# AutonomousVehicleLaboratory/vision_semantic_segmentation

Hardware: AMD Instinct MI355X
Metric: fused frames/sec/GPU (1920x1080 + 120k pts) + max|dlog-odds| vs ref (higher is better)
Workload: dtype f16 hi+lo split, MX-FP4 correction passes, fp32 accumulate

## Files before the change

### include/avl_hip.h

```cpp
#ifndef AVL_HIP_H
#define AVL_HIP_H

#include <stdint.h>

#ifdef __cplusplus
extern "C" {
#endif

#define AVL_OK 0
#define AVL_E_ARG (-1)
#define AVL_E_HIP (-2)
#define AVL_E_UNSUPPORTED (-3)

#define AVL_F32 0
#define AVL_F64 1
#define AVL_BF16 2
#define AVL_F16 3

#define AVL_MAX_MAP_CLASSES 16

const char* avl_version(void);
int avl_last_error(char* buf, int len);


// ... 252 lines not shown
    int32_t bias_per_image;
    int32_t in_format;
    int32_t raw_batch;
    void* out2;
    void* out2_lo;
    int32_t out2_ld, n_split;
} avl_seg_op;

#define AVL_IN_U8_HWC 0
#define AVL_IN_F32_CHW 1

#define AVL_MX_IN_LO 1
#define AVL_MX_RES_LO 2
#define AVL_MX_OUT_LO 4

typedef struct avl_seg_plan avl_seg_plan;

int avl_seg_plan_create(const avl_seg_op* ops_host, int n_ops, avl_seg_plan** out_plan);
void avl_seg_plan_destroy(avl_seg_plan* plan);
int avl_seg_plan_run(avl_seg_plan* plan, void* stream);
int avl_seg_plan_capture(avl_seg_plan* plan, void* stream);
int avl_seg_plan_profile(avl_seg_plan* plan, void* stream, float* ms_host, double* flops_host, double* bytes_host);
int avl_seg_plan_num_ops(const avl_seg_plan* plan);
int avl_seg_plan_nonfinite(avl_seg_plan* plan, void* stream, unsigned long long* counts_host);

#define AVL_GEMM_PLAIN 0
#define AVL_GEMM_RING 1
#define AVL_GEMM_RING_MX 2
#define AVL_GEMM_MX_PIPE 3

typedef struct avl_gemm_route {
    int32_t kernel;
    int32_t dtype;
    int32_t tile_m, tile_n;
    int32_t wm, wn;
    int32_t mi;
    int32_t stages;
    int32_t nsub;
    int32_t io;
    int32_t ast;
    int32_t ext;
    int32_t late;
    int32_t launches;
    int32_t m_tiles, n_tiles;
    int32_t workgroups;
} avl_gemm_route;
// ... 8 lines not shown
```

### vision_semantic_segmentation_amd/csrc/seg_conv.hip

```cpp
#include "seg_types.h"
#include "seg_preprocess.h"

namespace avl {
namespace {

constexpr int kThreads = 256;

template <typename T, bool F32IN = false>
__global__ void __launch_bounds__(kThreads) k_stem(const unsigned char* __restrict__ img, int H, int W,
                                                  const float* __restrict__ w, const float* __restrict__ bias,
                                                  T* __restrict__ out, int OH, int OW, int out_ld) {
    const int idx = blockIdx.x * kThreads + threadIdx.x;
    if (idx >= OH * OW) return;
    img = image_base(img, (long long)H * W, F32IN ? 3 * (int)sizeof(float) : 3);
    out = image_base(out, (long long)OH * OW, out_ld);
    const int oy = idx / OW, ox = idx % OW;
    float acc[64];
#pragma unroll
    for (int c = 0; c < 64; ++c) acc[c] = bias[c];
    const float mean[3] = {0.485f, 0.456f, 0.406f}, stdv[3] = {0.229f, 0.224f, 0.225f};
    for (int ky = 0; ky < 7; ++ky) {
        const int iy = oy * 2 - 3 + ky;
        for (int kx = 0; kx < 7; ++kx) {
            const int ix = ox * 2 - 3 + kx;
// ... 426 lines not shown
            Vec8<T>::load(in + (long long)(r + G) * in_ld + c8 * 8, v1);
            Vec8<T>::load(in + (long long)(r + 2 * G) * in_ld + c8 * 8, v2);
            Vec8<T>::load(in + (long long)(r + 3 * G) * in_ld + c8 * 8, v3);
#pragma unroll
            for (int i = 0; i < 8; ++i) s[i] += (v0[i] + v1[i]) + (v2[i] + v3[i]);
        }
        for (; r < M; r += G) {
            float v[8];
            Vec8<T>::load(in + (long long)r * in_ld + c8 * 8, v);
#pragma unroll
            for (int i = 0; i < 8; ++i) s[i] += v[i];
        }
        Vec8<float>::store(partial + (long long)blockIdx.x * C + c8 * 8, s);
    }
}
__global__ void __launch_bounds__(kThreads) k_gap_final(const float* __restrict__ partial, int G, int C, int M,
                                                       float* __restrict__ out, int out_ld) {
    __shared__ float red[8][32];
    const int cl = threadIdx.x & 31, sl = threadIdx.x >> 5;
    const int c = blockIdx.x * 32 + cl;
    partial = image_base(partial, G, C);
    out = image_base(out, 1, out_ld);
    float s = 0.f;
    if (c < C)
        for (int g = sl; g < G; g += 8) s += partial[(long long)g * C + c];
    red[sl][cl] = s;
    __syncthreads();
    if (sl == 0 && c < C) {
        float t = 0.f;
#pragma unroll
        for (int k = 0; k < 8; ++k) t += red[k][cl];
        out[c] = t / (float)M;
    }
}

__global__ void __launch_bounds__(kThreads) k_gemv(const float* __restrict__ in, const float* __restrict__ w,
                                                  const float* __restrict__ bias, float* __restrict__ out, int N, int K, int relu,
                                                  int in_ld, int out_ld) {
    const int n = blockIdx.x * (kThreads / 64) + (threadIdx.x >> 6);
    const int lane = threadIdx.x & 63;
    if (n >= N) return;
    in = image_base(in, 1, in_ld);
    out = image_base(out, 1, out_ld);
    const float* wr = w + (long long)n * K;
    float s0 = 0.f, s1 = 0.f, s2 = 0.f, s3 = 0.f;
    if ((K & 3) == 0 && (reinterpret_cast<uintptr_t>(wr) & 15) == 0 && (reinterpret_cast<uintptr_t>(in) & 15) == 0) {
#pragma unroll 8
        for (int k = lane * 4; k < K; k += 256) {
// ... 372 lines not shown
```

### vision_semantic_segmentation_amd/csrc/seg_dwpw.hip

```cpp
#include "seg_types.h"

namespace avl {
namespace {

constexpr int TM = 128;
constexpr int TN = 256;
constexpr int A_STAGE = TM * 128;
constexpr int W_STAGE = TN * 128;
constexpr int LDS_W = 0, LDS_A = 2 * W_STAGE, LDS_P = LDS_A + 2 * A_STAGE;
constexpr int P_STEP = 8 * 6 * 8 * 4;

struct DwPwArgs {
    const void* X;
    const void* X_lo;
    const void* Wc;
    const float* bc;
    float* LG;
    unsigned char* labels;
    int ncls;
    int tiles_x;
    const void* W;
    const float* bias;
    const uint32_t* dwp;
    const int* order;
// ... 184 lines not shown
                        hi[nj * 4 + r] = fmaxf(acc[mi][2 + nj][r], 0.f);
                    }
                HT* cp = static_cast<HT*>(p.C) + (long long)m * p.ldc + nbase;
                Vec8<HT>::store(cp, lo);
                Vec8<HT>::store(cp + 8, hi);
                if constexpr (WSUB != 1) {
                    if (p.C_lo) {
#pragma unroll
                        for (int i = 0; i < 8; ++i) { lo[i] -= (float)(HT)lo[i]; hi[i] -= (float)(HT)hi[i]; }
                        HT* cl = static_cast<HT*>(p.C_lo) + (long long)m * p.ldc + nbase;
                        Vec8<HT>::store(cl, lo);
                        Vec8<HT>::store(cl + 8, hi);
                    }
                }
            }
        }
    }
}

constexpr int X_LDS_W = 0, X_LDS_AH = 2 * W_STAGE, X_LDS_AL = X_LDS_AH + 2 * A_STAGE, X_LDS_P = X_LDS_AL + A_STAGE;
constexpr int XP_RING = 4;
constexpr int FP_STEP = 8 * 10 * 8 * 4;

__global__ void __launch_bounds__(512) k_dwpw_x(DwPwArgs p) {
    constexpr int PSTEP = FP_STEP;
    typedef f16 HT;
    typedef typename Half16<HT>::v8 v8;
    extern __shared__ __attribute__((aligned(16))) char lds[];
    const int tid = threadIdx.x, lane = tid & 63;
    const int wave = __builtin_amdgcn_readfirstlane(tid >> 6);
    const int wm = wave >> 2, wn = wave & 3;
    const int nt = blockIdx.x % p.ntiles;
    const int bm = blockIdx.x / p.ntiles, slot = (bm & 7) * p.per_xcd + (bm >> 3);
    if (slot >= p.mtiles) return;
    dwpw_image(p);
    const int mt = p.order[slot];
    const int nk = p.K / 64;

    const uint4* psrc = reinterpret_cast<const uint4*>(p.dwp);
    uint4 pnext = make_uint4(0u, 0u, 0u, 0u);
    auto load_p = [&](int s) { if (tid < PSTEP / 16 && s < nk) pnext = psrc[s * (PSTEP / 16) + tid]; };
    auto store_p = [&](int s) { if (tid < PSTEP / 16 && s < nk) *reinterpret_cast<uint4*>(lds + X_LDS_P + (s & (XP_RING - 1)) * PSTEP + tid * 16) = pnext; };
    for (int s = 0; s < 3; ++s) { load_p(s); store_p(s); }

    const int chunk = tid & 7, r0 = tid >> 3;
    unsigned voff[2][9];
#pragma unroll
    for (int q = 0; q < 2; ++q) {
        const int m = mt * TM + r0 + q * 64;
        const int y = m / p.OW, x = m - y * p.OW;
#pragma unroll
        for (int t = 0; t < 9; ++t) {
            const int iy = y - p.pad + (t / 3) * p.dil, ix = x - p.pad + (t % 3) * p.dil;
            const bool ok = m < p.M && iy >= 0 && iy < p.H && ix >= 0 && ix < p.Wd;
            voff[q][t] = ok ? (unsigned)(((long long)iy * p.Wd + ix) * p.ldx + chunk * 8) * 2u : 0x7fffff00u;
        }
    }
    const int wchunk = tid & 7, wrow0 = tid >> 3;
    const __amdgpu_buffer_rsrc_t wrsrc = __builtin_amdgcn_make_buffer_rsrc(
        const_cast<char*>(static_cast<const char*>(p.W) + (long long)nt * TN * p.K * 4), 0, TN * p.K * 4, 0x00020000);
    int w_voff[4];
#pragma unroll
    for (int i = 0; i < 4; ++i) w_voff[i] = (wrow0 + 64 * i) * p.K * 4 + wchunk * 16;
    v4i wl[4];
    auto load_w = [&](int h) {
#pragma unroll
        for (int i = 0; i < 4; ++i) wl[i] = __builtin_amdgcn_raw_buffer_load_b128(wrsrc, w_voff[i], h * 128, 0);
    };
    auto store_w = [&](int h) {
#pragma unroll
        for (int i = 0; i < 4; ++i) {
            const int r = wrow0 + 64 * i;
            const int key = ((r >> 1) & 1) | (((r >> 4) & 3) << 1);
            *reinterpret_cast<v4i*>(lds + X_LDS_W + (h & 1) * W_STAGE + r * 128 + ((wchunk ^ key) << 4)) = wl[i];
        }
// ... 8 lines not shown
        a_key[mi] = row & 7;
    }
#pragma unroll
    for (int nj = 0; nj < 4; ++nj) {
        const int row = wn * 64 + (fr >> 2) * 16 + nj * 4 + (fr & 3);
        w_off[nj] = X_LDS_W + row * 128;
        w_key[nj] = ((row >> 1) & 1) | (((row >> 4) & 3) << 1);
    }
    f32x4 acc[4][4];
    {
        const int nb = nt * TN + wn * 64 + kq * 16;
#pragma unroll
        for (int nj = 0; nj < 4; ++nj) {
            const float4 b = *reinterpret_cast<const float4*>(p.bias + nb + 4 * nj);
#pragma unroll
            for (int mi = 0; mi < 4; ++mi) acc[mi][nj] = f32x4{b.x, b.y, b.z, b.w};
        }
    }

    v4i raw[2][9];
    const __amdgpu_buffer_rsrc_t xrsrc = __builtin_amdgcn_make_buffer_rsrc(const_cast<void*>(p.X), 0, (int)p.x_bytes, 0x00020000);
    auto load_taps = [&](int s, int q) {
#pragma unroll
        for (int t = 0; t < 9; ++t) raw[q][t] = __builtin_amdgcn_raw_buffer_load_b128(xrsrc, (int)voff[q][t], s * 128, 0);
    };

    auto produce_a = [&](int s, int q) {
        float o[8];
        const float* pf = reinterpret_cast<const float*>(lds + X_LDS_P + (s & (XP_RING - 1)) * PSTEP + chunk * (10 * 8 * 4));
        {
            const float4 b0 = *reinterpret_cast<const float4*>(pf + 9 * 8), b1 = *reinterpret_cast<const float4*>(pf + 9 * 8 + 4);
            o[0] = b0.x; o[1] = b0.y; o[2] = b0.z; o[3] = b0.w;
            o[4] = b1.x; o[5] = b1.y; o[6] = b1.z; o[7] = b1.w;
        }
        typedef _Float16 h2 __attribute__((ext_vector_type(2)));
#pragma unroll
        for (int t = 0; t < 9; ++t) {
            const float4 w0 = *reinterpret_cast<const float4*>(pf + t * 8), w1 = *reinterpret_cast<const float4*>(pf + t * 8 + 4);
            const float wt[8] = {w0.x, w0.y, w0.z, w0.w, w1.x, w1.y, w1.z, w1.w};
#pragma unroll
            for (int j = 0; j < 4; ++j) {
                const int u = raw[q][t][j];
                const h2 v = __builtin_bit_cast(h2, u);
                o[2 * j] = __builtin_fmaf((float)v[0], wt[2 * j], o[2 * j]);
                o[2 * j + 1] = __builtin_fmaf((float)v[1], wt[2 * j + 1], o[2 * j + 1]);
            }
        }
        float ol[8];
#pragma unroll
        for (int i = 0; i < 8; ++i) {
            o[i] = fmaxf(o[i], 0.f);
            ol[i] = o[i] - (float)(HT)o[i];
        }
        const int row = r0 + q * 64;
        const int sw = row * 128 + ((chunk ^ (row & 7)) << 4);
        Vec8<HT>::store(reinterpret_cast<HT*>(lds + X_LDS_AH + (s & 1) * A_STAGE + sw), o);
        Vec8<HT>::store(reinterpret_cast<HT*>(lds + X_LDS_AL + sw), ol);
    };

    load_taps(0, 0);
// ... 64 lines not shown
                float lo[8], hi[8];
#pragma unroll
                for (int nj = 0; nj < 2; ++nj)
#pragma unroll
                    for (int r = 0; r < 4; ++r) {
                        lo[nj * 4 + r] = fmaxf(acc[mi][nj][r], 0.f);
                        hi[nj * 4 + r] = fmaxf(acc[mi][2 + nj][r], 0.f);
                    }
                HT* cp = static_cast<HT*>(p.C) + (long long)m * p.ldc + nbase;
                Vec8<HT>::store(cp, lo);
                Vec8<HT>::store(cp + 8, hi);
                if (p.C_lo) {
#pragma unroll
                    for (int i = 0; i < 8; ++i) { lo[i] -= (float)(HT)lo[i]; hi[i] -= (float)(HT)hi[i]; }
                    HT* cl = static_cast<HT*>(p.C_lo) + (long long)m * p.ldc + nbase;
                    Vec8<HT>::store(cl, lo);
                    Vec8<HT>::store(cl + 8, hi);
                }
            }
        }
    }
}

int launch_dwpw_x(const DwPwArgs& a, hipStream_t s) {
    constexpr int lds_bytes = X_LDS_P + XP_RING * FP_STEP;
    static_assert(lds_bytes <= 160 * 1024, "k_dwpw_x LDS");
    AVL_HIP_CHECK(hipFuncSetAttribute(reinterpret_cast<const void*>(&k_dwpw_x), hipFuncAttributeMaxDynamicSharedMemorySize, 160 * 1024));
    hipLaunchKernelGGL(k_dwpw_x, dim3(8 * a.per_xcd * a.ntiles, 1, a.nimg), dim3(512), lds_bytes, s, a);
    AVL_LAUNCH_CHECK();
    return AVL_OK;
}

constexpr int S_LDS_W = 0, S_LDS_AH = 2 * W_STAGE, S_LDS_AL = S_LDS_AH + 2 * A_STAGE, S_LDS_P = S_LDS_AL + 2 * A_STAGE;
template <bool CLS>
__global__ void __launch_bounds__(512) k_dwpw_xs(DwPwArgs p) {
    constexpr int PSTEP = FP_STEP;
    typedef f16 HT;
    typedef typename Half16<HT>::v8 v8;
    extern __shared__ __attribute__((aligned(16))) char lds[];
    const int tid = threadIdx.x, lane = tid & 63;
    const int wave = __builtin_amdgcn_readfirstlane(tid >> 6);
    const int wm = wave >> 2, wn = wave & 3;
    const int nt = blockIdx.x % p.ntiles;
    const int bm = blockIdx.x / p.ntiles, slot = (bm & 7) * p.per_xcd + (bm >> 3);
    if (slot >= p.mtiles) return;
    dwpw_image(p);
    const int mt = p.order[slot];
    const int nk = p.K / 64;

    const unsigned lds0 = lds_addr(lds);
    auto dma_p = [&](int s) {
// ... 334 lines not shown
                    "dwpw with out_f32 (classifier + arg-max in the epilogue): needs a split input, w_split 3, out_c 256, in3 = f16 [2][32][256] weights, in2_lo = "
                    "fp32 bias[32], out = fp32 logits [rows][in3_c <= 32] (out_ld = in3_c), out_mx = uint8 labels[rows], no out_lo");
        AVL_REQUIRE((reinterpret_cast<uintptr_t>(op.in3) | reinterpret_cast<uintptr_t>(op.in2_lo)) % 16 == 0 && reinterpret_cast<uintptr_t>(op.out) % 4 == 0, "dwpw classifier operands unaligned");
    }
    AVL_REQUIRE(op.w_split != 2, "dwpw: w_split 2 (f16 depthwise weight pairs) was replaced by w_split 3 (fp32 depthwise weights)");
    AVL_REQUIRE(!op.in_lo || op.w_split == 3, "dwpw: a split input (in_lo) needs the exact depthwise stage (w_split 3: k_dwpw_xs)");
    AVL_REQUIRE(op.w_layout == 0 || (op.w_layout == 1 && op.in_lo && op.w_split == 3), "dwpw: w_layout 1 (8 x 16-pixel tiles) exists for the split-input kernel only");
    AVL_REQUIRE((reinterpret_cast<uintptr_t>(op.out_lo) | reinterpret_cast<uintptr_t>(op.in_lo)) % 16 == 0, "dwpw low planes must be 16-byte aligned");
    const int M = op.out_h * op.out_w, K = op.in_c, N = op.out_c;
    AVL_REQUIRE(op.stride == 1 && op.ksize == 3 && op.dil >= 1 && op.pad >= 0 && op.out_h == op.in_h + 2 * op.pad - 2 * op.dil &&
                    op.out_w == op.in_w + 2 * op.pad - 2 * op.dil && M > 0,
                "dwpw geometry: 3x3, stride 1, output = input + 2 pad - 2 dilation");
    AVL_REQUIRE(K % 64 == 0 && K <= 2048, "dwpw K = %d (multiple of 64, <= 2048: the depthwise parameters live in LDS)", K);
    AVL_REQUIRE(N % 16 == 0 && op.w_rows >= (N + TN - 1) / TN * TN, "dwpw N = %d / weight rows %d", N, op.w_rows);
    AVL_REQUIRE(op.in_ld >= K && (op.in_ld * 2) % 16 == 0, "dwpw in_ld %d", op.in_ld);
    if (!op.out_f32) AVL_REQUIRE(op.out_ld >= N && (op.out_ld * 2) % 16 == 0, "dwpw out_ld %d", op.out_ld);
    AVL_REQUIRE(op.in_rows >= op.in_h * op.in_w * op_batch(op) && op.out_rows >= M * op_batch(op), "dwpw rows");
    AVL_REQUIRE((long long)op.in_rows * op.in_ld * 2 < 0x7fffff00LL, "dwpw input larger than a buffer descriptor's range");
    AVL_REQUIRE((reinterpret_cast<uintptr_t>(op.in) | reinterpret_cast<uintptr_t>(op.weight) | reinterpret_cast<uintptr_t>(op.out) |
                 reinterpret_cast<uintptr_t>(op.bias) | reinterpret_cast<uintptr_t>(op.in2)) % 16 == 0, "dwpw buffers must be 16-byte aligned");
    return AVL_OK;
}

int launch_dwpw(const avl_seg_op& op, hipStream_t s) {
    DwPwArgs a;
    a.X = op.in; a.X_lo = op.in_lo; a.W = op.weight;
    a.Wc = nullptr; a.bc = nullptr; a.LG = nullptr; a.labels = nullptr; a.ncls = 0;
    a.tiles_x = (op.w_layout == 1) ? (op.out_w + 15) / 16 : 0; a.bias = op.bias; a.dwp = static_cast<const uint32_t*>(op.in2); a.C = op.out;
    a.H = op.in_h; a.Wd = op.in_w; a.OW = op.out_w; a.ldx = op.in_ld; a.ldc = op.out_ld; a.pad = op.pad;
    a.M = op.out_h * op.out_w; a.N = op.out_c; a.K = op.in_c; a.dil = op.dil;
    a.ntiles = (a.N + TN - 1) / TN;
    a.x_bytes = (unsigned)((long long)op.in_rows * op.in_ld * 2);
    a.nimg = op_batch(op);
    const int mtiles = a.tiles_x > 0 ? a.tiles_x * ((op.out_h + 7) / 8) : (a.M + TM - 1) / TM;
    a.mtiles = mtiles;
    a.per_xcd = (mtiles + 7) / 8;
    a.order = reinterpret_cast<const int*>(a.dwp + (a.K / 64) * ((op.w_split == 3 ? FP_STEP : P_STEP) / 4));
    a.C_lo = op.out_lo;
    if (op.w_split == 3 && op.out_f32) {
        a.Wc = op.in3; a.bc = static_cast<const float*>(op.in2_lo); a.LG = static_cast<float*>(op.out); a.labels = static_cast<unsigned char*>(op.out_mx);
        a.ncls = op.in3_c;
        return launch_dwpw_xs<true>(a, s);
    }
    if (op.w_split == 3) return op.in_lo ? launch_dwpw_xs<false>(a, s) : launch_dwpw_x(a, s);
    if (op.w_split) return launch_dwpw_typed<f16, 2>(a, mtiles, s);
    return op.dtype == AVL_F16 ? launch_dwpw_typed<f16, 1>(a, mtiles, s) : launch_dwpw_typed<bf16, 1>(a, mtiles, s);
}

}
```

### vision_semantic_segmentation_amd/csrc/seg_plan.hip

```cpp
#include <vector>

#include "seg_types.h"

struct avl_seg_plan {
    std::vector<avl_seg_op> ops;
    std::vector<hipEvent_t> ev;
    hipGraph_t graph = nullptr;
    hipGraphExec_t exec = nullptr;
};

namespace avl {
namespace {

int validate(const avl_seg_op& op, int index) {
    int rc;
    if (op.batch < 0) rc = set_error(AVL_E_ARG, "batch %d (0 or 1 = one image)", op.batch);
    else if (op.bias_per_image && op.kind != AVL_OP_GEMM) rc = set_error(AVL_E_ARG, "bias_per_image is a GEMM field");
    else if (op.in_format != AVL_IN_U8_HWC && op.in_format != AVL_IN_F32_CHW) rc = set_error(AVL_E_ARG, "in_format %d is not an AVL_IN_* value", op.in_format);
    else if (op.in_format != AVL_IN_U8_HWC && op.kind != AVL_OP_STEM) rc = set_error(AVL_E_ARG, "in_format %d is a stem field (other ops leave it 0)", op.in_format);
    else if (op.in_format == AVL_IN_F32_CHW && op.in2)
        rc = set_error(AVL_E_UNSUPPORTED, op.raw_batch ? "in_format AVL_IN_F32_CHW with raw_batch = 1: a batch of raw frames is uint8 [batch][src_h][src_w][3]"
                                                       : "in_format AVL_IN_F32_CHW with a pre-processing stem (in2 set): that stem reads the raw uint8 frame");
    else if (op.raw_batch != 0 && op.raw_batch != 1) rc = set_error(AVL_E_ARG, "raw_batch %d (0 = one raw frame, 1 = every image of the batch is a raw frame)", op.raw_batch);
    else if (op.raw_batch && op.kind != AVL_OP_STEM) rc = set_error(AVL_E_ARG, "raw_batch is a stem field (other ops leave it 0)");
    else if (op.raw_batch && !op.in2) rc = set_error(AVL_E_ARG, "raw_batch needs a pre-processing stem: in2 (the camera blocks) is NULL");
    else if (op.kind == AVL_OP_GEMM) rc = validate_gemm(op);
    else if (op.kind == AVL_OP_DWPW) rc = validate_dwpw(op);
    else if (op.kind == AVL_OP_BOTTLENECK) rc = validate_bottleneck(op);
    else rc = validate_conv_op(op);
    if (rc != AVL_OK) {
        char msg[400];
        snprintf(msg, sizeof(msg), "%s", err_buf());
        return set_error(rc, "op %d (kind %d): %s", index, op.kind, msg);
    }
    return AVL_OK;
}

int launch(const avl_seg_op& op, hipStream_t s) {
    if (op.kind == AVL_OP_GEMM) return launch_gemm(op, s);
    if (op.kind == AVL_OP_DWPW) return launch_dwpw(op, s);
    if (op.kind == AVL_OP_BOTTLENECK) return launch_bottleneck(op, s);
    return launch_conv_op(op, s);
}

static double act_bytes(double es, bool lo_plane, bool mx, bool mx_lo) {
    double b = es + (lo_plane ? es : 0.0);
    if (mx) b += (mx_lo ? 2.0 : 1.0) * (0.5 + 1.0 / 32.0);
    return b;
}

void work(const avl_seg_op& op, double& flops, double& bytes) {
    const double es = elem_size(op.dtype), nb = op_batch(op);
    const double in_pix = (double)op.in_h * op.in_w * nb, out_pix = (double)op.out_h * op.out_w * nb;
    const double e_in = act_bytes(es, op.in_lo != nullptr, op.in_mx != nullptr, (op.mx_flags & AVL_MX_IN_LO) || op.in_lo);
    const double e_out = act_bytes(es, op.out_lo != nullptr, op.out_mx != nullptr, (op.mx_flags & AVL_MX_OUT_LO) || op.out_lo);
    flops = 0;
    bytes = in_pix * op.in_c * e_in + out_pix * op.out_c * e_out;
    switch (op.kind) {
        case AVL_OP_STEM:
            flops = 2.0 * (op.stride == 4 ? nb * ((op.in_h - 1) / 2 + 1) * ((op.in_w - 1) / 2 + 1) : out_pix) * 64 * 147;
            bytes = (op.in2 ? (double)op.in_rows : in_pix) * (op.in_format == AVL_IN_F32_CHW ? 12 : 3) + out_pix * 64 * es;
            break;
        case AVL_OP_GEMM:
            flops = 2.0 * out_pix * op.out_c * (op.in_c + (op.in3 ? op.in3_c : 0));
            {
                const double k_all = op.in_c + (op.in3 ? op.in3_c : 0);
                const double e_w = op.w_split == 2 ? es + 2.0 * (0.5 + 1.0 / 32.0) : es * (op.w_split ? 2.0 : 1.0);
// ... 39 lines not shown
        case AVL_OP_GEMV:
            flops = 2.0 * op.in_c * op.out_c * nb;
            bytes = 4.0 * op.in_c * op.out_c + 4.0 * (op.in_c + op.out_c) * nb;
            break;
        case AVL_OP_ARGMAX:
            bytes = in_pix * op.in_c * 4 + in_pix;
            break;
        default:
            break;
    }
}

}
}

extern "C" int avl_seg_plan_create(const avl_seg_op* ops_host, int n_ops, avl_seg_plan** out_plan) {
    AVL_REQUIRE(ops_host && n_ops > 0 && out_plan, "avl_seg_plan_create: bad arguments");
    for (int i = 0; i < n_ops; ++i) {
        int rc = avl::validate(ops_host[i], i);
        if (rc) return rc;
    }
    avl_seg_plan* p = new avl_seg_plan();
    p->ops.assign(ops_host, ops_host + n_ops);
    *out_plan = p;
    return AVL_OK;
}

extern "C" void avl_seg_plan_destroy(avl_seg_plan* plan) {
    if (!plan) return;
    if (plan->exec) (void)hipGraphExecDestroy(plan->exec);
    if (plan->graph) (void)hipGraphDestroy(plan->graph);
    for (hipEvent_t e : plan->ev) (void)hipEventDestroy(e);
    delete plan;
}

extern "C" int avl_seg_plan_num_ops(const avl_seg_plan* plan) { return plan ? (int)plan->ops.size() : 0; }

extern "C" int avl_seg_plan_capture(avl_seg_plan* plan, void* stream) {
    AVL_REQUIRE(plan && stream, "avl_seg_plan_capture needs a plan and a non-NULL stream");
    hipStream_t s = avl::as_stream(stream);
    if (plan->exec) { (void)hipGraphExecDestroy(plan->exec); plan->exec = nullptr; }
    if (plan->graph) { (void)hipGraphDestroy(plan->graph); plan->graph = nullptr; }
    AVL_HIP_CHECK(hipStreamBeginCapture(s, hipStreamCaptureModeThreadLocal));
    int rc = AVL_OK;
    for (const avl_seg_op& op : plan->ops) {
        rc = avl::launch(op, s);
        if (rc) break;
    }
    hipGraph_t g = nullptr;
    hipError_t e = hipStreamEndCapture(s, &g);
    if (rc) { if (g) (void)hipGraphDestroy(g); return rc; }
    if (e != hipSuccess) return avl::set_error(AVL_E_HIP, "hipStreamEndCapture failed: %s", hipGetErrorString(e));
    plan->graph = g;
    AVL_HIP_CHECK(hipGraphInstantiate(&plan->exec, plan->graph, nullptr, nullptr, 0));
    return AVL_OK;
}

extern "C" int avl_seg_plan_run(avl_seg_plan* plan, void* stream) {
    AVL_REQUIRE(plan, "plan is NULL");
    hipStream_t s = avl::as_stream(stream);
    if (plan->exec) {
        AVL_HIP_CHECK(hipGraphLaunch(plan->exec, s));
        return AVL_OK;
    }
    for (const avl_seg_op& op : plan->ops) {
        int rc = avl::launch(op, s);
        if (rc) return rc;
    }
    return AVL_OK;
}

extern "C" int avl_seg_plan_profile(avl_seg_plan* plan, void* stream, float* ms_host, double* flops_host, double* bytes_host) {
    AVL_REQUIRE(plan && ms_host, "avl_seg_plan_profile: bad arguments");
    hipStream_t s = avl::as_stream(stream);
    const size_t n = plan->ops.size();
    while (plan->ev.size() < 2 * n) {
        hipEvent_t e;
        AVL_HIP_CHECK(hipEventCreate(&e));
        plan->ev.push_back(e);
    }
    for (size_t i = 0; i < n; ++i) {
        AVL_HIP_CHECK(hipEventRecord(plan->ev[2 * i], s));
        int rc = avl::launch(plan->ops[i], s);
        if (rc) return rc;
        AVL_HIP_CHECK(hipEventRecord(plan->ev[2 * i + 1], s));
    }
    AVL_HIP_CHECK(hipStreamSynchronize(s));
    for (size_t i = 0; i < n; ++i) {
        AVL_HIP_CHECK(hipEventElapsedTime(&ms_host[i], plan->ev[2 * i], plan->ev[2 * i + 1]));
        double f, b;
        avl::work(plan->ops[i], f, b);
        if (flops_host) flops_host[i] = f;
        if (bytes_host) bytes_host[i] = b;
    }
    return AVL_OK;
}

namespace avl {
namespace {
template <typename T>
__global__ void k_count_nonfinite(const T* x, long long rows, int cols, int ld, unsigned long long* counter) {
    const long long n = rows * cols;
    unsigned long long bad = 0;
    for (long long i = (long long)blockIdx.x * blockDim.x + threadIdx.x; i < n; i += (long long)gridDim.x * blockDim.x) {
        const float v = (float)x[(i / cols) * ld + (i % cols)];
        bad += (__builtin_isfinite(v) ? 0u : 1u);
    }
    for (int o = 32; o > 0; o >>= 1) bad += __shfl_down(bad, o, 64);
    if ((threadIdx.x & 63) == 0 && bad) atomicAdd(counter, bad);
}
template <typename T>
void count_plane(const void* ptr, long long rows, int cols, int ld, unsigned long long* counter, hipStream_t s) {
// ... 75 lines not shown
```

### vision_semantic_segmentation_amd/csrc/seg_types.h

```cpp
#pragma once
#include <hip/hip_runtime.h>

#include "avl_common.h"

namespace avl {

typedef __bf16 bf16;
typedef __bf16 bf16x8 __attribute__((ext_vector_type(8)));
typedef _Float16 f16;
typedef _Float16 f16x8 __attribute__((ext_vector_type(8)));
typedef float f32x4 __attribute__((ext_vector_type(4)));
typedef float f32x8 __attribute__((ext_vector_type(8)));

template <typename T>
struct Vec8;

template <>
struct Vec8<bf16> {
    static __device__ __forceinline__ void load(const bf16* p, float (&v)[8]) {
        const bf16x8 x = *reinterpret_cast<const bf16x8*>(p);
#pragma unroll
        for (int i = 0; i < 8; ++i) v[i] = (float)x[i];
    }
    static __device__ __forceinline__ void store(bf16* p, const float (&v)[8]) {
// ... 157 lines not shown
__host__ __device__ inline long long mx_scale_bytes(long long rows, long long channels) { return (channels / 256) * rows * 8; }
template <typename C>
inline MxBundle<C> mx_bundle_at(C* b, long long rows, long long channels) {
    const long long P = mx_plane_bytes(rows, channels), S = mx_scale_bytes(rows, channels);
    return {{b, b + P + S}, {b + P, b + 2 * P + S}, (int)(channels / 2), rows};
}
inline MxBundle<char> mx_bundle(void* base, long long rows, long long channels) { return mx_bundle_at(static_cast<char*>(base), rows, channels); }
inline MxBundle<const char> mx_bundle(const void* base, long long rows, long long channels) { return mx_bundle_at(static_cast<const char*>(base), rows, channels); }

int launch_gemm(const avl_seg_op& op, hipStream_t s);
int validate_gemm(const avl_seg_op& op);
int launch_conv_op(const avl_seg_op& op, hipStream_t s);
int validate_conv_op(const avl_seg_op& op);
int launch_gconv_mfma(const avl_seg_op& op, hipStream_t s);
int validate_gconv_mfma(const avl_seg_op& op);
int launch_conv3x3(const avl_seg_op& op, hipStream_t s);
int validate_conv3x3(const avl_seg_op& op);
int launch_stem_mfma(const avl_seg_op& op, hipStream_t s);
int launch_stem_pre_f32(const avl_seg_op& op, hipStream_t s);
int launch_dwconv_k(const avl_seg_op& op, hipStream_t s);
int validate_dwconv_k(const avl_seg_op& op);
int launch_dwpw(const avl_seg_op& op, hipStream_t s);
int validate_dwpw(const avl_seg_op& op);
int launch_bottleneck(const avl_seg_op& op, hipStream_t s);
int validate_bottleneck(const avl_seg_op& op);

}
```

### vision_semantic_segmentation_amd/network.py

```python
import collections
import ctypes as C
import hashlib
import math

import numpy as np
import torch

from . import _lib

BN_EPS = 1e-5

OP_STEM, OP_MAXPOOL, OP_GEMM, OP_GCONV, OP_DWCONV, OP_BILINEAR, OP_GAP, OP_GEMV, OP_ARGMAX, OP_SUBSAMPLE, OP_DWPW, OP_BOTTLENECK = range(1, 13)
OP_NAMES = {1: "stem", 2: "maxpool", 3: "gemm", 4: "gconv", 5: "dwconv", 6: "bilinear", 7: "gap", 8: "gemv", 9: "argmax", 10: "subsample", 11: "dwpw",
            12: "bottleneck"}


class AvlSegOp(C.Structure):
    _fields_ = [
        ("kind", C.c_int32), ("dtype", C.c_int32),
        ("in_", C.c_void_p), ("in2", C.c_void_p), ("out", C.c_void_p), ("weight", C.c_void_p), ("bias", C.c_void_p),
        ("in_h", C.c_int32), ("in_w", C.c_int32), ("in_c", C.c_int32), ("in_ld", C.c_int32), ("in_rows", C.c_int32),
        ("out_h", C.c_int32), ("out_w", C.c_int32), ("out_c", C.c_int32), ("out_ld", C.c_int32), ("out_rows", C.c_int32),
        ("in2_ld", C.c_int32),
        ("ksize", C.c_int32), ("stride", C.c_int32), ("pad", C.c_int32), ("dil", C.c_int32), ("groups", C.c_int32),
# ... 30 lines not shown
    d = {name: getattr(r, name) for name, _ in AvlGemmRoute._fields_}
    d["kernel"] = GEMM_KERNELS[r.kernel]
    return d


def gemm_kernel_name(route):
    t = {_lib.AVL_F32: "float", _lib.AVL_BF16: "bf16", _lib.AVL_F16: "f16"}[route["dtype"]]
    args = {"k_gemm": [t, "wm", "wn"],
            "k_gemm_ring": [t, "wm", "wn", "mi", "stages", "nsub", "io", "ast", "true" if route["ext"] else "false"],
            "k_gemm_ring_mx": ["io", "mi"],
            "k_gemm_mx_pipe": ["io", "mi", "late"]}[route["kernel"]]
    return "%s<%s>" % (route["kernel"], ", ".join(str(route.get(a, a)) for a in args))


_vp, _i = C.c_void_p, C.c_int
_lib._register_seg({
    "avl_seg_gemm_route": (_i, [C.POINTER(AvlSegOp), C.POINTER(AvlGemmRoute)]),
    "avl_seg_plan_create": (_i, [C.POINTER(AvlSegOp), _i, C.POINTER(C.c_void_p)]),
    "avl_seg_plan_destroy": (None, [_vp]),
    "avl_seg_plan_run": (_i, [_vp, _vp]),
    "avl_seg_plan_capture": (_i, [_vp, _vp]),
    "avl_seg_plan_profile": (_i, [_vp, _vp, _vp, _vp, _vp]),
    "avl_seg_plan_num_ops": (_i, [_vp]),
    "avl_seg_plan_nonfinite": (_i, [_vp, _vp, _vp]),
})


PLANES = (64, 128, 256, 512)
EXPANSION = 4
BACKBONES = {
    "resnet50": ((3, 4, 6, 3), 1, 64),
    "resnet101": ((3, 4, 23, 3), 1, 64),
    "resnet152": ((3, 8, 36, 3), 1, 64),
    "resnext50_32x4d": ((3, 4, 6, 3), 32, 4),
    "resnext101_32x8d": ((3, 4, 23, 3), 32, 8),
    "wide_resnet50_2": ((3, 4, 6, 3), 1, 128),
    "wide_resnet101_2": ((3, 4, 23, 3), 1, 128),
}
DEFAULT_BACKBONE = "resnext50_32x4d"
UNBUILDABLE_BACKBONES = ("ResNet", "resnet18", "resnet34")
LAYERS, GROUPS, WIDTH_PER_GROUP = BACKBONES[DEFAULT_BACKBONE]


def backbone_arch(name):
    if name in BACKBONES:
        return BACKBONES[name]
# ... 1102 lines not shown
            if self.input_format == "f32_nchw":
                if tuple(image_u8.shape) != tuple(self.image.shape) or not image_u8.dtype.is_floating_point:
                    raise ValueError("this plan takes a float tensor of shape %s, not %s %s" % (tuple(self.image.shape), image_u8.dtype,
                                                                                               tuple(image_u8.shape)))
            else:
                if self.raw_batch and self.batch == 1 and image_u8.dim() == 4:
                    image_u8 = image_u8[0]
                assert tuple(image_u8.shape) == tuple(self.image.shape) and image_u8.dtype == torch.uint8
            self.image.copy_(image_u8, non_blocking=True)
        s = torch.cuda.current_stream(self.device).cuda_stream if stream is None else stream
        _lib.check(_lib.lib().avl_seg_plan_run(self._plan, C.c_void_p(s)), "avl_seg_plan_run")
        return self.labels if hasattr(self, "labels_buf") else None

    def capture_graph(self):
        side = torch.cuda.Stream(device=self.device)
        side.wait_stream(torch.cuda.current_stream(self.device))
        with torch.cuda.stream(side):
            _lib.check(_lib.lib().avl_seg_plan_run(self._plan, C.c_void_p(side.cuda_stream)), "avl_seg_plan_run")
            side.synchronize()
            _lib.check(_lib.lib().avl_seg_plan_capture(self._plan, C.c_void_p(side.cuda_stream)), "avl_seg_plan_capture")
        torch.cuda.current_stream(self.device).wait_stream(side)
        self.graphed = True

    def profile(self):
        n = len(self.ops)
        ms, fl, by = (C.c_float * n)(), (C.c_double * n)(), (C.c_double * n)()
        s = torch.cuda.current_stream(self.device).cuda_stream
        _lib.check(_lib.lib().avl_seg_plan_profile(self._plan, C.c_void_p(s), ms, fl, by), "avl_seg_plan_profile")
        return [dict(name=self.op_names[i], kind=OP_NAMES[self.ops[i].kind], ms=ms[i], flops=fl[i], bytes=by[i]) for i in range(n)]

    def op_output(self, i):
        op = self.ops[i]
        rows, cols = op.out_h * op.out_w * self.batch, (op.in3_c if (op.kind == OP_DWPW and op.out_f32) else (op.n_split if op.out2 else op.out_c))
        dt = torch.float32 if (op.out_f32 or op.dtype == _lib.AVL_F32) else self.act_dtype

        def plane(ptr):
            for t in self._keep + ([self.logits_buf] if hasattr(self, "logits_buf") else []):
                lo, hi = t.data_ptr(), t.data_ptr() + t.numel() * t.element_size()
                if lo <= ptr < hi:
                    flat = t.reshape(-1).view(torch.uint8)[ptr - lo:].view(dt)
                    return torch.as_strided(flat, (rows, cols), (op.out_ld, 1)).float().cpu()
            raise KeyError("op %d: output pointer not in the plan's buffers" % i)
        y = plane(op.out)
        return y + plane(op.out_lo) if op.out_lo else y

    def run_prefix(self, n_ops, stream=None):
# ... 21 lines not shown
```

Measured before the change: 229.8.

## Group sibling dwpw ops into one launch with border-aware tap skipping

Consecutive depthwise+pointwise ops that share the same input and have non-overlapping outputs (likely the ASPP dilated branches) are merged into a single kernel launch. A host-built dispatch table spreads the interior (all-taps-live) tiles evenly across the XCDs. The tile kernel is templated on whether the top or bottom tap row falls entirely outside the image, so those loads and FMAs are dropped at compile time. The GAP final reduction is also unrolled to keep 32 loads in flight. The cost is a device table built on the first run, a requirement that the plan runs once before graph capture, and larger kernel arguments.

Result: no change. 231.3 (median of 6 runs) (+0.7%).

```diff
diff --git a/include/avl_hip.h b/include/avl_hip.h
--- a/include/avl_hip.h
+++ b/include/avl_hip.h
@@ -298,6 +298,7 @@
 int avl_seg_plan_capture(avl_seg_plan* plan, void* stream);
 int avl_seg_plan_profile(avl_seg_plan* plan, void* stream, float* ms_host, double* flops_host, double* bytes_host);
 int avl_seg_plan_num_ops(const avl_seg_plan* plan);
+int avl_seg_plan_launch_of(const avl_seg_plan* plan, int* launch_of_op_host);
 int avl_seg_plan_nonfinite(avl_seg_plan* plan, void* stream, unsigned long long* counts_host);
 
 #define AVL_GEMM_PLAIN 0
diff --git a/vision_semantic_segmentation_amd/csrc/seg_conv.hip b/vision_semantic_segmentation_amd/csrc/seg_conv.hip
--- a/vision_semantic_segmentation_amd/csrc/seg_conv.hip
+++ b/vision_semantic_segmentation_amd/csrc/seg_conv.hip
@@ -472,8 +472,17 @@
     partial = image_base(partial, G, C);
     out = image_base(out, 1, out_ld);
     float s = 0.f;
-    if (c < C)
-        for (int g = sl; g < G; g += 8) s += partial[(long long)g * C + c];
+    if (c < C) {
+        int g = sl;
+        for (; g + 8 * 31 < G; g += 8 * 32) {
+            float v[32];
+#pragma unroll
+            for (int i = 0; i < 32; ++i) v[i] = partial[(long long)(g + 8 * i) * C + c];
+#pragma unroll
+            for (int i = 0; i < 32; ++i) s += v[i];
+        }
+        for (; g < G; g += 8) s += partial[(long long)g * C + c];
+    }
     red[sl][cl] = s;
     __syncthreads();
     if (sl == 0 && c < C) {
diff --git a/vision_semantic_segmentation_amd/csrc/seg_dwpw.hip b/vision_semantic_segmentation_amd/csrc/seg_dwpw.hip
--- a/vision_semantic_segmentation_amd/csrc/seg_dwpw.hip
+++ b/vision_semantic_segmentation_amd/csrc/seg_dwpw.hip
@@ -1,3 +1,7 @@
+#include <algorithm>
+#include <utility>
+#include <vector>
+
 #include "seg_types.h"
 
 namespace avl {
@@ -230,19 +234,15 @@
 constexpr int XP_RING = 4;
 constexpr int FP_STEP = 8 * 10 * 8 * 4;
 
-__global__ void __launch_bounds__(512) k_dwpw_x(DwPwArgs p) {
+template <bool TOP, bool BOT>
+__device__ __forceinline__ void dwpw_x_tile(const DwPwArgs& p, const int mt, const int nt, char* lds) {
     constexpr int PSTEP = FP_STEP;
     typedef f16 HT;
     typedef typename Half16<HT>::v8 v8;
-    extern __shared__ __attribute__((aligned(16))) char lds[];
+    auto dead = [](int t) { return (TOP && t / 3 == 0) || (BOT && t / 3 == 2); };
     const int tid = threadIdx.x, lane = tid & 63;
     const int wave = __builtin_amdgcn_readfirstlane(tid >> 6);
     const int wm = wave >> 2, wn = wave & 3;
-    const int nt = blockIdx.x % p.ntiles;
-    const int bm = blockIdx.x / p.ntiles, slot = (bm & 7) * p.per_xcd + (bm >> 3);
-    if (slot >= p.mtiles) return;
-    dwpw_image(p);
-    const int mt = p.order[slot];
     const int nk = p.K / 64;
 
     const uint4* psrc = reinterpret_cast<const uint4*>(p.dwp);
@@ -259,6 +259,7 @@
         const int y = m / p.OW, x = m - y * p.OW;
 #pragma unroll
         for (int t = 0; t < 9; ++t) {
+            if (dead(t)) continue;
             const int iy = y - p.pad + (t / 3) * p.dil, ix = x - p.pad + (t % 3) * p.dil;
             const bool ok = m < p.M && iy >= 0 && iy < p.H && ix >= 0 && ix < p.Wd;
             voff[q][t] = ok ? (unsigned)(((long long)iy * p.Wd + ix) * p.ldx + chunk * 8) * 2u : 0x7fffff00u;
@@ -313,7 +314,8 @@
     const __amdgpu_buffer_rsrc_t xrsrc = __builtin_amdgcn_make_buffer_rsrc(const_cast<void*>(p.X), 0, (int)p.x_bytes, 0x00020000);
     auto load_taps = [&](int s, int q) {
 #pragma unroll
-        for (int t = 0; t < 9; ++t) raw[q][t] = __builtin_amdgcn_raw_buffer_load_b128(xrsrc, (int)voff[q][t], s * 128, 0);
+        for (int t = 0; t < 9; ++t)
+            if (!dead(t)) raw[q][t] = __builtin_amdgcn_raw_buffer_load_b128(xrsrc, (int)voff[q][t], s * 128, 0);
     };
 
     auto produce_a = [&](int s, int q) {
@@ -327,6 +329,7 @@
         typedef _Float16 h2 __attribute__((ext_vector_type(2)));
 #pragma unroll
         for (int t = 0; t < 9; ++t) {
+            if (dead(t)) continue;
             const float4 w0 = *reinterpret_cast<const float4*>(pf + t * 8), w1 = *reinterpret_cast<const float4*>(pf + t * 8 + 4);
             const float wt[8] = {w0.x, w0.y, w0.z, w0.w, w1.x, w1.y, w1.z, w1.w};
 #pragma unroll
@@ -437,11 +440,42 @@
     }
 }
 
-int launch_dwpw_x(const DwPwArgs& a, hipStream_t s) {
+struct DwPwGroup {
+    DwPwArgs m[DWPW_GROUP_MAX];
+    const unsigned* table;
+    int n;
+};
+
+__global__ void __launch_bounds__(512) k_dwpw_x(DwPwGroup g) {
+    extern __shared__ __attribute__((aligned(16))) char lds[];
+    const int ntiles = g.m[0].ntiles, per_xcd = g.m[0].per_xcd;
+    const int nt = blockIdx.x % ntiles;
+    const int bm = blockIdx.x / ntiles;
+    int gi = 0, slot = (bm & 7) * per_xcd + (bm >> 3);
+    if (g.table) {
+        const unsigned e = g.table[(bm & 7) * (g.n * per_xcd) + (bm >> 3)];
+        gi = __builtin_amdgcn_readfirstlane((int)(e >> 24));
+        slot = __builtin_amdgcn_readfirstlane((int)(e & 0xffffffu));
+    }
+    DwPwArgs p = g.m[gi];
+    if (slot >= p.mtiles) return;
+    dwpw_image(p);
+    const int mt = p.order[slot];
+    const int m_last = min(mt * TM + TM, p.M) - 1;
+    const bool top = m_last / p.OW - p.pad < 0, bot = (mt * TM) / p.OW - p.pad + 2 * p.dil >= p.H;
+    if (top && bot) dwpw_x_tile<true, true>(p, mt, nt, lds);
+    else if (top) dwpw_x_tile<true, false>(p, mt, nt, lds);
+    else if (bot) dwpw_x_tile<false, true>(p, mt, nt, lds);
+    else dwpw_x_tile<false, false>(p, mt, nt, lds);
+}
+
+int launch_dwpw_x(const DwPwGroup& g, hipStream_t s) {
     constexpr int lds_bytes = X_LDS_P + XP_RING * FP_STEP;
     static_assert(lds_bytes <= 160 * 1024, "k_dwpw_x LDS");
+    static_assert(sizeof(DwPwGroup) <= 2048, "k_dwpw_x kernel arguments");
+    const DwPwArgs& a = g.m[0];
     AVL_HIP_CHECK(hipFuncSetAttribute(reinterpret_cast<const void*>(&k_dwpw_x), hipFuncAttributeMaxDynamicSharedMemorySize, 160 * 1024));
-    hipLaunchKernelGGL(k_dwpw_x, dim3(8 * a.per_xcd * a.ntiles, 1, a.nimg), dim3(512), lds_bytes, s, a);
+    hipLaunchKernelGGL(k_dwpw_x, dim3(g.n * 8 * a.per_xcd * a.ntiles, 1, a.nimg), dim3(512), lds_bytes, s, g);
     AVL_LAUNCH_CHECK();
     return AVL_OK;
 }
@@ -822,8 +856,104 @@
     return AVL_OK;
 }
 
-int launch_dwpw(const avl_seg_op& op, hipStream_t s) {
-    DwPwArgs a;
+namespace {
+
+bool dwpw_x_route(const avl_seg_op& op) { return op.kind == AVL_OP_DWPW && op.w_split == 3 && !op.in_lo && !op.out_f32; }
+
+bool planes_apart(const void* pa, long long rows_a, int ld_a, const void* pb, long long rows_b, int ld_b, int n) {
+    if (!pa || !pb) return true;
+    const uintptr_t a = reinterpret_cast<uintptr_t>(pa), b = reinterpret_cast<uintptr_t>(pb);
+    const uintptr_t ea = a + (uintptr_t)rows_a * ld_a * 2, eb = b + (uintptr_t)rows_b * ld_b * 2;
+    if (ea <= b || eb <= a) return true;
+    if (ld_a != ld_b) return false;
+    const uintptr_t ld = (uintptr_t)ld_a * 2, d = (a > b ? a - b : b - a) % ld, w = (uintptr_t)n * 2;
+    return d >= w && d + w <= ld;
+}
+
+void dwpw_args(const avl_seg_op& op, DwPwArgs& a);
+
+}
+
+bool dwpw_can_group(const avl_seg_op& a, const avl_seg_op& b) {
+    if (!dwpw_x_route(a) || !dwpw_x_route(b)) return false;
+    if (a.in != b.in || a.in_h != b.in_h || a.in_w != b.in_w || a.in_c != b.in_c || a.in_ld != b.in_ld || a.in_rows != b.in_rows) return false;
+    if (a.out_h != b.out_h || a.out_w != b.out_w || a.out_c != b.out_c || a.dtype != b.dtype || op_batch(a) != op_batch(b)) return false;
+    const void* outs_a[2] = {a.out, a.out_lo};
+    const void* outs_b[2] = {b.out, b.out_lo};
+    for (const void* pa : outs_a)
+        for (const void* pb : outs_b)
+            if (!planes_apart(pa, a.out_rows, a.out_ld, pb, b.out_rows, b.out_ld, a.out_c)) return false;
+    for (const void* pa : outs_a)
+        if (!planes_apart(pa, a.out_rows, a.out_ld, a.in, a.in_rows, a.in_ld, std::max(a.in_c, a.out_c))) return false;
+    for (const void* pb : outs_b)
+        if (!planes_apart(pb, b.out_rows, b.out_ld, a.in, a.in_rows, a.in_ld, std::max(a.in_c, a.out_c))) return false;
+    return true;
+}
+
+int dwpw_group_table(const avl_seg_op* ops, int n, unsigned** table_dev) {
+    AVL_REQUIRE(ops && n >= 2 && n <= DWPW_GROUP_MAX && table_dev, "dwpw group of %d", n);
+    DwPwArgs a0;
+    dwpw_args(ops[0], a0);
+    const int per_xcd = a0.per_xcd, mtiles = a0.mtiles;
+    std::vector<std::vector<int>> cls(n, std::vector<int>(8 * per_xcd, 3));
+    std::vector<int> order(mtiles);
+    for (int g = 0; g < n; ++g) {
+        DwPwArgs a;
+        dwpw_args(ops[g], a);
+        AVL_REQUIRE(a.mtiles == mtiles && a.per_xcd == per_xcd && a.ntiles == a0.ntiles && a.nimg == a0.nimg, "dwpw group: member %d has another grid", g);
+        AVL_HIP_CHECK(hipMemcpy(order.data(), a.order, sizeof(int) * mtiles, hipMemcpyDeviceToHost));
+        for (int slot = 0; slot < mtiles; ++slot) {
+            const int mt = order[slot];
+            if (mt < 0 || mt >= mtiles) continue;
+            const int m_last = std::min(mt * TM + TM, a.M) - 1;
+            cls[g][slot] = (m_last / a.OW - a.pad < 0 ? 1 : 0) + ((mt * TM) / a.OW - a.pad + 2 * a.dil >= a.H ? 1 : 0);
+        }
+    }
+    typedef std::pair<int, unsigned> Entry;
+    std::vector<std::vector<Entry>> row(8);
+    int live_all = 0;
+    for (int xcd = 0; xcd < 8; ++xcd) {
+        for (int c = 0; c < 4; ++c)
+            for (int g = 0; g < n; ++g)
+                for (int j = 0; j < per_xcd; ++j)
+                    if (cls[g][xcd * per_xcd + j] == c) row[xcd].push_back(Entry(c, (unsigned)g << 24 | (unsigned)(xcd * per_xcd + j)));
+        live_all += (int)std::count_if(row[xcd].begin(), row[xcd].end(), [](const Entry& e) { return e.first == 0; });
+    }
+    const int share = (live_all + 7) / 8;
+    auto live = [&](int x) { return (int)std::count_if(row[x].begin(), row[x].end(), [](const Entry& e) { return e.first == 0; }); };
+    for (int x = 0; x < 8; ++x)
+        for (int y = 0; y < 8 && live(x) > share; ++y)
+            while (live(x) > share && live(y) < share) std::swap(row[x][live(x) - 1], row[y][live(y)]);
+    std::vector<unsigned> table;
+    std::vector<char> seen((size_t)n * 8 * per_xcd, 0);
+    for (int xcd = 0; xcd < 8; ++xcd) {
+        std::stable_sort(row[xcd].begin(), row[xcd].end(), [](const Entry& a, const Entry& b) { return a.first < b.first; });
+        for (const Entry& e : row[xcd]) {
+            table.push_back(e.second);
+            seen[(size_t)(e.second >> 24) * 8 * per_xcd + (e.second & 0xffffffu)] = 1;
+        }
+        AVL_REQUIRE((int)row[xcd].size() == n * per_xcd, "dwpw group table: a row of %d entries", (int)row[xcd].size());
+    }
+    AVL_REQUIRE(std::count(seen.begin(), seen.end(), 1) == (long)seen.size(), "dwpw group table: not every slot of every member is dispatched once");
+    unsigned* dev = nullptr;
+    AVL_HIP_CHECK(hipMalloc(reinterpret_cast<void**>(&dev), table.size() * sizeof(unsigned)));
+    hipError_t e = hipMemcpy(dev, table.data(), table.size() * sizeof(unsigned), hipMemcpyHostToDevice);
+    if (e != hipSuccess) { (void)hipFree(dev); return set_error(AVL_E_HIP, "dwpw group table: %s", hipGetErrorString(e)); }
+    *table_dev = dev;
+    return AVL_OK;
+}
+
+int launch_dwpw_group(const avl_seg_op* ops, int n, const unsigned* table_dev, hipStream_t s) {
+    AVL_REQUIRE(ops && n >= 2 && n <= DWPW_GROUP_MAX && table_dev, "dwpw group of %d", n);
+    DwPwGroup g;
+    for (int i = 0; i < DWPW_GROUP_MAX; ++i) dwpw_args(ops[i < n ? i : 0], g.m[i]);
+    g.table = table_dev;
+    g.n = n;
+    return launch_dwpw_x(g, s);
+}
+
+namespace {
+void dwpw_args(const avl_seg_op& op, DwPwArgs& a) {
     a.X = op.in; a.X_lo = op.in_lo; a.W = op.weight;
     a.Wc = nullptr; a.bc = nullptr; a.LG = nullptr; a.labels = nullptr; a.ncls = 0;
     a.tiles_x = (op.w_layout == 1) ? (op.out_w + 15) / 16 : 0; a.bias = op.bias; a.dwp = static_cast<const uint32_t*>(op.in2); a.C = op.out;
@@ -832,17 +962,30 @@
     a.ntiles = (a.N + TN - 1) / TN;
     a.x_bytes = (unsigned)((long long)op.in_rows * op.in_ld * 2);
     a.nimg = op_batch(op);
-    const int mtiles = a.tiles_x > 0 ? a.tiles_x * ((op.out_h + 7) / 8) : (a.M + TM - 1) / TM;
-    a.mtiles = mtiles;
-    a.per_xcd = (mtiles + 7) / 8;
+    a.mtiles = a.tiles_x > 0 ? a.tiles_x * ((op.out_h + 7) / 8) : (a.M + TM - 1) / TM;
+    a.per_xcd = (a.mtiles + 7) / 8;
     a.order = reinterpret_cast<const int*>(a.dwp + (a.K / 64) * ((op.w_split == 3 ? FP_STEP : P_STEP) / 4));
     a.C_lo = op.out_lo;
+}
+}
+
+int launch_dwpw(const avl_seg_op& op, hipStream_t s) {
+    DwPwArgs a;
+    dwpw_args(op, a);
+    const int mtiles = a.mtiles;
     if (op.w_split == 3 && op.out_f32) {
         a.Wc = op.in3; a.bc = static_cast<const float*>(op.in2_lo); a.LG = static_cast<float*>(op.out); a.labels = static_cast<unsigned char*>(op.out_mx);
         a.ncls = op.in3_c;
         return launch_dwpw_xs<true>(a, s);
     }
-    if (op.w_split == 3) return op.in_lo ? launch_dwpw_xs<false>(a, s) : launch_dwpw_x(a, s);
+    if (op.w_split == 3 && !op.in_lo) {
+        DwPwGroup g;
+        for (DwPwArgs& m : g.m) m = a;
+        g.table = nullptr;
+        g.n = 1;
+        return launch_dwpw_x(g, s);
+    }
+    if (op.w_split == 3) return launch_dwpw_xs<false>(a, s);
     if (op.w_split) return launch_dwpw_typed<f16, 2>(a, mtiles, s);
     return op.dtype == AVL_F16 ? launch_dwpw_typed<f16, 1>(a, mtiles, s) : launch_dwpw_typed<bf16, 1>(a, mtiles, s);
 }
diff --git a/vision_semantic_segmentation_amd/csrc/seg_plan.hip b/vision_semantic_segmentation_amd/csrc/seg_plan.hip
--- a/vision_semantic_segmentation_amd/csrc/seg_plan.hip
+++ b/vision_semantic_segmentation_amd/csrc/seg_plan.hip
@@ -1,9 +1,15 @@
 #include <vector>
 
 #include "seg_types.h"
+
+struct avl_seg_launch {
+    int first = 0, n = 1;
+    unsigned* table = nullptr;
+};
 
 struct avl_seg_plan {
     std::vector<avl_seg_op> ops;
+    std::vector<avl_seg_launch> launches;
     std::vector<hipEvent_t> ev;
     hipGraph_t graph = nullptr;
     hipGraphExec_t exec = nullptr;
@@ -43,6 +49,18 @@
     return launch_conv_op(op, s);
 }
 
+int launch(avl_seg_plan* plan, avl_seg_launch& l, hipStream_t s) {
+    if (l.n == 1) return launch(plan->ops[l.first], s);
+    if (!l.table) {
+        hipStreamCaptureStatus cap = hipStreamCaptureStatusNone;
+        AVL_HIP_CHECK(hipStreamIsCapturing(s, &cap));
+        AVL_REQUIRE(cap == hipStreamCaptureStatusNone, "the plan has to run once before it is captured (a launch group makes its dispatch table on its first launch)");
+        int rc = dwpw_group_table(&plan->ops[l.first], l.n, &l.table);
+        if (rc) return rc;
+    }
+    return launch_dwpw_group(&plan->ops[l.first], l.n, l.table, s);
+}
+
 static double act_bytes(double es, bool lo_plane, bool mx, bool mx_lo) {
     double b = es + (lo_plane ? es : 0.0);
     if (mx) b += (mx_lo ? 2.0 : 1.0) * (0.5 + 1.0 / 32.0);
@@ -128,12 +146,33 @@
     }
     avl_seg_plan* p = new avl_seg_plan();
     p->ops.assign(ops_host, ops_host + n_ops);
+    for (int i = 0; i < n_ops;) {
+        avl_seg_launch l;
+        l.first = i;
+        while (l.n < avl::DWPW_GROUP_MAX && i + l.n < n_ops) {
+            bool ok = true;
+            for (int j = i; j < i + l.n && ok; ++j) ok = avl::dwpw_can_group(p->ops[j], p->ops[i + l.n]);
+            if (!ok) break;
+            ++l.n;
+        }
+        p->launches.push_back(l);
+        i += l.n;
+    }
     *out_plan = p;
     return AVL_OK;
+}
+
+extern "C" int avl_seg_plan_launch_of(const avl_seg_plan* plan, int* launch_of_op_host) {
+    if (!plan) return 0;
+    for (size_t l = 0; launch_of_op_host && l < plan->launches.size(); ++l)
+        for (int j = 0; j < plan->launches[l].n; ++j) launch_of_op_host[plan->launches[l].first + j] = (int)l;
+    return (int)plan->launches.size();
 }
 
 extern "C" void avl_seg_plan_destroy(avl_seg_plan* plan) {
     if (!plan) return;
+    for (avl_seg_launch& l : plan->launches)
+        if (l.table) (void)hipFree(l.table);
     if (plan->exec) (void)hipGraphExecDestroy(plan->exec);
     if (plan->graph) (void)hipGraphDestroy(plan->graph);
     for (hipEvent_t e : plan->ev) (void)hipEventDestroy(e);
@@ -149,8 +188,8 @@
     if (plan->graph) { (void)hipGraphDestroy(plan->graph); plan->graph = nullptr; }
     AVL_HIP_CHECK(hipStreamBeginCapture(s, hipStreamCaptureModeThreadLocal));
     int rc = AVL_OK;
-    for (const avl_seg_op& op : plan->ops) {
-        rc = avl::launch(op, s);
+    for (avl_seg_launch& l : plan->launches) {
+        rc = avl::launch(plan, l, s);
         if (rc) break;
     }
     hipGraph_t g = nullptr;
@@ -169,8 +208,8 @@
         AVL_HIP_CHECK(hipGraphLaunch(plan->exec, s));
         return AVL_OK;
     }
-    for (const avl_seg_op& op : plan->ops) {
-        int rc = avl::launch(op, s);
+    for (avl_seg_launch& l : plan->launches) {
+        int rc = avl::launch(plan, l, s);
         if (rc) return rc;
     }
     return AVL_OK;
@@ -185,15 +224,19 @@
         AVL_HIP_CHECK(hipEventCreate(&e));
         plan->ev.push_back(e);
     }
+    for (avl_seg_launch& l : plan->launches) {
+        AVL_HIP_CHECK(hipEventRecord(plan->ev[2 * l.first], s));
+        int rc = avl::launch(plan, l, s);
+        if (rc) return rc;
+        AVL_HIP_CHECK(hipEventRecord(plan->ev[2 * l.first + 1], s));
+    }
+    AVL_HIP_CHECK(hipStreamSynchronize(s));
+    for (const avl_seg_launch& l : plan->launches) {
+        float ms = 0.f;
+        AVL_HIP_CHECK(hipEventElapsedTime(&ms, plan->ev[2 * l.first], plan->ev[2 * l.first + 1]));
+        for (int j = 0; j < l.n; ++j) ms_host[l.first + j] = ms / l.n;
+    }
     for (size_t i = 0; i < n; ++i) {
-        AVL_HIP_CHECK(hipEventRecord(plan->ev[2 * i], s));
-        int rc = avl::launch(plan->ops[i], s);
-        if (rc) return rc;
-        AVL_HIP_CHECK(hipEventRecord(plan->ev[2 * i + 1], s));
-    }
-    AVL_HIP_CHECK(hipStreamSynchronize(s));
-    for (size_t i = 0; i < n; ++i) {
-        AVL_HIP_CHECK(hipEventElapsedTime(&ms_host[i], plan->ev[2 * i], plan->ev[2 * i + 1]));
         double f, b;
         avl::work(plan->ops[i], f, b);
         if (flops_host) flops_host[i] = f;
diff --git a/vision_semantic_segmentation_amd/csrc/seg_types.h b/vision_semantic_segmentation_amd/csrc/seg_types.h
--- a/vision_semantic_segmentation_amd/csrc/seg_types.h
+++ b/vision_semantic_segmentation_amd/csrc/seg_types.h
@@ -203,6 +203,10 @@
 int validate_dwconv_k(const avl_seg_op& op);
 int launch_dwpw(const avl_seg_op& op, hipStream_t s);
 int validate_dwpw(const avl_seg_op& op);
+constexpr int DWPW_GROUP_MAX = 4;
+bool dwpw_can_group(const avl_seg_op& a, const avl_seg_op& b);
+int dwpw_group_table(const avl_seg_op* ops, int n, unsigned** table_dev);
+int launch_dwpw_group(const avl_seg_op* ops, int n, const unsigned* table_dev, hipStream_t s);
 int launch_bottleneck(const avl_seg_op& op, hipStream_t s);
 int validate_bottleneck(const avl_seg_op& op);
 
diff --git a/vision_semantic_segmentation_amd/network.py b/vision_semantic_segmentation_amd/network.py
--- a/vision_semantic_segmentation_amd/network.py
+++ b/vision_semantic_segmentation_amd/network.py
@@ -76,6 +76,7 @@
     "avl_seg_plan_capture": (_i, [_vp, _vp]),
     "avl_seg_plan_profile": (_i, [_vp, _vp, _vp, _vp, _vp]),
     "avl_seg_plan_num_ops": (_i, [_vp]),
+    "avl_seg_plan_launch_of": (_i, [_vp, _vp]),
     "avl_seg_plan_nonfinite": (_i, [_vp, _vp, _vp]),
 })
 
@@ -1224,6 +1225,12 @@
         torch.cuda.current_stream(self.device).wait_stream(side)
         self.graphed = True
 
+    def launch_of(self):
+        n = len(self.ops)
+        out = (C.c_int * n)()
+        _lib.lib().avl_seg_plan_launch_of(self._plan, out)
+        return list(out)
+
     def profile(self):
         n = len(self.ops)
         ms, fl, by = (C.c_float * n)(), (C.c_double * n)(), (C.c_double * n)()
```
